# yeyupiaoling/MASR

Measured on NVIDIA H100. Metric: audio_seconds_per_second, higher is better.
Workload: dtype f32 (GEMMs: fp16x2-split operands on wgmma, fp32 accumulate; fp32-grade results)

## Files before the change

### masr_b200/csrc/ffn_tc.cu

```cuda
#include <cuda.h>
#include <cuda_fp16.h>
#include <string.h>

#include "tc_common.cuh"

namespace masr {

namespace {

constexpr int FM = 64;
constexpr int FD = 256;
constexpr int FHC = 128;
constexpr int FBK = 32;
constexpr int F_STAGES = 4;
constexpr int F_STAGE_BYTES = 32768;
constexpr int F_H_BYTES = FM * FHC * 2 * 2;
constexpr int F_SUM_BYTES = FM * FD * 4;
constexpr int F_THREADS = 384;
constexpr int F_PRODUCER_REGS = 40, F_CONSUMER_REGS = 232;
constexpr uint32_t F_TX_A = 2 * FM * FBK * 2 + 2 * FHC * FBK * 2;
constexpr uint32_t F_TX_B = 2 * FD * FBK * 2;
constexpr size_t kFfnSmem = F_STAGES * F_STAGE_BYTES + F_H_BYTES + F_SUM_BYTES + 1024 + 256;
static_assert(kFfnSmem <= 232448, "ffn_tc shared memory exceeds the 227 KB per-CTA limit of sm_90");
static_assert(F_PRODUCER_REGS * 128 + F_CONSUMER_REGS * 256 <= 65536, "register file of the SM");

struct FfnMaps {
    CUtensorMap xh, xl;
    CUtensorMap w1h, w1l;
    CUtensorMap w2h, w2l;
};

struct FfnParams {
    const float* b1;
    const float* b2;
    float* x;
    int64_t ldx;
    int M, F;
    float alpha;
};

__device__ __forceinline__ void wgmma_m64n64k16_ss(float (&d)[32], uint64_t da, uint64_t db, uint32_t scale_d) {
    asm volatile(
        "{\n\t"
        ".reg .pred p;\n\t"
        "setp.ne.b32 p, %34, 0;\n\t"
        "wgmma.mma_async.sync.aligned.m64n64k16.f32.f16.f16 "
        "{%0, %1, %2, %3, %4, %5, %6, %7, %8, %9, %10, %11, %12, %13, %14, %15, "
        "%16, %17, %18, %19, %20, %21, %22, %23, %24, %25, %26, %27, %28, %29, %30, %31}, %32, %33, p, 1, 1, 0, 0;\n\t"
        "}"
        : "+f"(d[0]), "+f"(d[1]), "+f"(d[2]), "+f"(d[3]), "+f"(d[4]), "+f"(d[5]), "+f"(d[6]), "+f"(d[7]), "+f"(d[8]),
          "+f"(d[9]), "+f"(d[10]), "+f"(d[11]), "+f"(d[12]), "+f"(d[13]), "+f"(d[14]), "+f"(d[15]), "+f"(d[16]),
          "+f"(d[17]), "+f"(d[18]), "+f"(d[19]), "+f"(d[20]), "+f"(d[21]), "+f"(d[22]), "+f"(d[23]), "+f"(d[24]),
          "+f"(d[25]), "+f"(d[26]), "+f"(d[27]), "+f"(d[28]), "+f"(d[29]), "+f"(d[30]), "+f"(d[31])
        : "l"(da), "l"(db), "r"(scale_d));
}

__device__ __forceinline__ void bar_consumers() { asm volatile("bar.sync 1, 256;" ::: "memory"); }

__global__ void __launch_bounds__(F_THREADS, 1) ffn_tc_kernel(const __grid_constant__ FfnMaps maps, FfnParams p) {
    extern __shared__ uint8_t smem_raw[];
    uint8_t* smem = reinterpret_cast<uint8_t*>((reinterpret_cast<uintptr_t>(smem_raw) + 1023) & ~uintptr_t(1023));
    uint8_t* hbuf = smem + F_STAGES * F_STAGE_BYTES;
    uint8_t* sum = hbuf + F_H_BYTES;
    uint64_t* full_bar = reinterpret_cast<uint64_t*>(sum + F_SUM_BYTES);
    uint64_t* empty_bar = full_bar + F_STAGES;

    const int warp = threadIdx.x >> 5, lane = threadIdx.x & 31;
    const int nrb = (p.M + FM - 1) / FM;
    const int nch = p.F / FHC;

    if (warp == 8 && lane == 0) {
        tma_prefetch_desc(&maps.xh); tma_prefetch_desc(&maps.xl); tma_prefetch_desc(&maps.w1h);
        tma_prefetch_desc(&maps.w1l); tma_prefetch_desc(&maps.w2h); tma_prefetch_desc(&maps.w2l);
        for (int s = 0; s < F_STAGES; ++s) { mbar_init(&full_bar[s], 1); mbar_init(&empty_bar[s], 8); }
        asm volatile("fence.mbarrier_init.release.cluster;" ::: "memory");
    }
    __syncthreads();
    pdl_wait();
    pdl_launch_dependents();

    if (warp >= 8) {
        setmaxnreg_dec<F_PRODUCER_REGS>();
        if (warp == 8 && elect_one_sync()) {
            uint32_t kg = 0;
            auto acquire = [&](uint32_t tx) {
                const uint32_t s = kg % F_STAGES;
                mbar_wait(&empty_bar[s], ((kg / F_STAGES) & 1) ^ 1);
                mbar_expect_tx(&full_bar[s], tx);
                ++kg;
                return s;
            };
            for (int rb = blockIdx.x; rb < nrb; rb += gridDim.x) {
                const int m0 = rb * FM;
                for (int j = -1; j < nch; ++j) {
                    if (j >= 0) {
#pragma unroll 1
                        for (int kb = 0; kb < FHC / FBK; ++kb) {
                            const uint32_t s = acquire(F_TX_B);
                            uint8_t* st = smem + s * F_STAGE_BYTES;
                            tma_load_2d(&maps.w2h, &full_bar[s], st, j * FHC + kb * FBK, 0);
                            tma_load_2d(&maps.w2l, &full_bar[s], st + F_STAGE_BYTES / 2, j * FHC + kb * FBK, 0);
                        }
                    }
                    if (j + 1 < nch) {
#pragma unroll 1
                        for (int kb = 0; kb < FD / FBK; ++kb) {
                            const uint32_t s = acquire(F_TX_A);
                            uint8_t* st = smem + s * F_STAGE_BYTES;
                            tma_load_2d(&maps.xh, &full_bar[s], st, kb * FBK, m0);
                            tma_load_2d(&maps.xl, &full_bar[s], st + 4096, kb * FBK, m0);
                            tma_load_2d(&maps.w1h, &full_bar[s], st + 8192, kb * FBK, (j + 1) * FHC);
                            tma_load_2d(&maps.w1l, &full_bar[s], st + 16384, kb * FBK, (j + 1) * FHC);
                        }
                    }
                }
            }
        }
        __syncwarp();
    } else {
        setmaxnreg_inc<F_CONSUMER_REGS>();
        const int wg = warp >> 2, wi = warp & 3, q = lane & 3;
        const int tid = threadIdx.x & 127;
        const uint32_t h_base = smem_u32(hbuf);
        const uint32_t sum_base = smem_u32(sum) + wg * (F_SUM_BYTES / 2) + tid * 8;
        const uint32_t is_lane0 = lane == 0;
        auto release = [&](uint32_t s) {
            asm volatile("{\n\t.reg .pred p;\n\tsetp.ne.u32 p, %1, 0;\n\t@p mbarrier.arrive.shared::cta.b64 _, [%0];\n\t}"
                         ::"r"(smem_u32(&empty_bar[s])), "r"(is_lane0) : "memory");
        };
        float acc1[32], cor1[32], acc2[64], cor2[64];
        uint32_t kg = 0;
        int pend = -1;
        auto next_stage = [&]() {
            const uint32_t s = kg % F_STAGES;
            mbar_wait(&full_bar[s], (kg / F_STAGES) & 1);
            ++kg;
            return s;
        };
        auto retire = [&](uint32_t s) {
            wgmma_wait<1>();
            reg_fence(acc1); reg_fence(cor1); reg_fence(acc2); reg_fence(cor2);
            if (pend >= 0) release((uint32_t)pend);
            pend = (int)s;
        };
        auto phase_a = [&]() {
#pragma unroll 1
            for (int kb = 0; kb < FD / FBK; ++kb) {
                const uint32_t s = next_stage();
                const uint32_t sa = smem_u32(smem + s * F_STAGE_BYTES);
                const uint64_t dXh = gmma_desc_sw64(sa), dXl = gmma_desc_sw64(sa + 4096);
                const uint64_t dWh = gmma_desc_sw64(sa + 8192 + wg * 4096), dWl = gmma_desc_sw64(sa + 16384 + wg * 4096);
                reg_fence(acc1); reg_fence(cor1);
                wgmma_fence();
#pragma unroll
                for (int ks = 0; ks < FBK / 16; ++ks) {
                    const uint64_t adv = (uint64_t)(ks * 2);
                    const uint32_t first = (kb | ks) ? 1u : 0u;
                    wgmma_m64n64k16_ss(acc1, dXh + adv, dWh + adv, first);
                    wgmma_m64n64k16_ss(cor1, dXh + adv, dWl + adv, first);
                    wgmma_m64n64k16_ss(cor1, dXl + adv, dWh + adv, 1u);
                }
                wgmma_commit();
                retire(s);
            }
        };
        auto phase_b = [&](int j) {
#pragma unroll 1
            for (int kb = 0; kb < FHC / FBK; ++kb) {
                const uint32_t s = next_stage();
                const uint32_t sa = smem_u32(smem + s * F_STAGE_BYTES);
                const uint64_t dWh = gmma_desc_sw64(sa + wg * 8192), dWl = gmma_desc_sw64(sa + F_STAGE_BYTES / 2 + wg * 8192);
                const uint64_t dHh = gmma_desc_sw64(h_base + kb * 8192), dHl = gmma_desc_sw64(h_base + kb * 8192 + 4096);
                reg_fence(acc2); reg_fence(cor2);
                wgmma_fence();
#pragma unroll
                for (int ks = 0; ks < FBK / 16; ++ks) {
                    const uint64_t adv = (uint64_t)(ks * 2);
                    wgmma_m64n128k16_ss(acc2, dHh + adv, dWh + adv, ((j & 1) | kb | ks) ? 1u : 0u);
                    wgmma_m64n128k16_ss(cor2, dHh + adv, dWl + adv, (j | kb | ks) ? 1u : 0u);
                    wgmma_m64n128k16_ss(cor2, dHl + adv, dWh + adv, 1u);
                }
                wgmma_commit();
                retire(s);
            }
        };
        const int r_lo = 16 * wi + (lane >> 2);
        auto store_hidden = [&](int j) {
            float2 bb[8];
            const float* b = p.b1 + j * FHC + 64 * wg + 2 * q;
#pragma unroll
            for (int i = 0; i < 8; ++i) bb[i] = __ldg(reinterpret_cast<const float2*>(b + 8 * i));
#pragma unroll
            for (int i = 0; i < 8; ++i)
#pragma unroll
                for (int hh = 0; hh < 2; ++hh) {
                    float v0 = fmaf(cor1[4 * i + 2 * hh], kLoInv, acc1[4 * i + 2 * hh]);
                    float v1 = fmaf(cor1[4 * i + 2 * hh + 1], kLoInv, acc1[4 * i + 2 * hh + 1]);
                    v0 += bb[i].x; v1 += bb[i].y;
                    float e0, e1;
                    mul2(e0, e1, v0, v1, -1.4426950408889634f, -1.4426950408889634f);
                    e0 = ex2_approx(e0); e1 = ex2_approx(e1);
                    add2(e0, e1, e0, e1, 1.0f, 1.0f);
                    e0 = rcp_approx(e0); e1 = rcp_approx(e1);
                    mul2(v0, v1, v0, v1, e0, e1);
                    __half2 h2, l2;
                    split_f16x2(v0, v1, h2, l2);
                    const int r = r_lo + 8 * hh, c = 64 * wg + 8 * i + 2 * q;
                    const uint32_t a = h_base + (c >> 5) * 8192 + r * 64 + ((((c & 31) >> 3) ^ ((r >> 1) & 3)) << 4) + (c & 7) * 2;
                    asm volatile("st.shared.b32 [%0], %1;" ::"r"(a), "r"(*reinterpret_cast<uint32_t*>(&h2)) : "memory");
                    asm volatile("st.shared.b32 [%0], %1;" ::"r"(a + 4096), "r"(*reinterpret_cast<uint32_t*>(&l2)) : "memory");
                }
            asm volatile("fence.proxy.async.shared::cta;" ::: "memory");
        };
        auto drain = [&]() {
            wgmma_wait<0>();
            reg_fence(acc1); reg_fence(cor1); reg_fence(acc2); reg_fence(cor2);
            if (pend >= 0) release((uint32_t)pend);
            pend = -1;
        };

        for (int rb = blockIdx.x; rb < nrb; rb += gridDim.x) {
            const int m0 = rb * FM;
            phase_a();
            drain();
            bar_consumers();
            store_hidden(0);
            bar_consumers();
#pragma unroll 1
            for (int j = 0; j < nch; ++j) {
                phase_b(j);
                if (j + 1 < nch) phase_a();
                drain();
                if ((j & 1) && j + 1 < nch) {
#pragma unroll
                    for (int i = 0; i < 16; ++i)
#pragma unroll
                        for (int hh = 0; hh < 2; ++hh) {
                            float x0 = acc2[4 * i + 2 * hh], x1 = acc2[4 * i + 2 * hh + 1];
                            const uint32_t a = sum_base + (i * 2 + hh) * 1024;
                            if (j > 1) {
                                float s0, s1;
                                asm volatile("ld.shared.v2.f32 {%0, %1}, [%2];" : "=f"(s0), "=f"(s1) : "r"(a) : "memory");
                                x0 = s0 + x0; x1 = s1 + x1;
                            }
                            asm volatile("st.shared.v2.f32 [%0], {%1, %2};" ::"r"(a), "f"(x0), "f"(x1) : "memory");
                        }
                }
                if (j + 1 < nch) {
                    bar_consumers();
                    store_hidden(j + 1);
                    bar_consumers();
                }
            }
            const float* b2 = p.b2 + 128 * wg + 2 * q;
#pragma unroll
            for (int i = 0; i < 16; ++i) {
                const float2 bv = __ldg(reinterpret_cast<const float2*>(b2 + 8 * i));
#pragma unroll
                for (int hh = 0; hh < 2; ++hh) {
                    float x0 = acc2[4 * i + 2 * hh], x1 = acc2[4 * i + 2 * hh + 1];
                    if (nch > 2) {
                        float s0, s1;
                        asm volatile("ld.shared.v2.f32 {%0, %1}, [%2];" : "=f"(s0), "=f"(s1) : "r"(sum_base + (i * 2 + hh) * 1024) : "memory");
                        x0 = s0 + x0; x1 = s1 + x1;
                    }
                    x0 = fmaf(cor2[4 * i + 2 * hh], kLoInv, x0);
                    x1 = fmaf(cor2[4 * i + 2 * hh + 1], kLoInv, x1);
                    x0 += bv.x; x1 += bv.y;
                    const int row = m0 + r_lo + 8 * hh;
                    if (row < p.M) {
                        float2* xp = reinterpret_cast<float2*>(p.x + (int64_t)row * p.ldx + 128 * wg + 8 * i + 2 * q);
                        const float2 r = *xp;
                        x0 = r.x + p.alpha * x0;
                        x1 = r.y + p.alpha * x1;
                        *xp = make_float2(x0, x1);
                    }
                }
            }
        }
    }
    __syncthreads();
}

int ffn_map(CUtensorMap* map, const void* ptr, int64_t rows, int64_t K, int64_t ld, int box_rows) {
    EncodeTiledFn fn = get_encode_fn();
    if (!fn) { set_last_error("cuTensorMapEncodeTiled entry point unavailable"); return MASR_ERR_INTERNAL; }
    cuuint64_t dims[2] = {(cuuint64_t)K, (cuuint64_t)rows};
    cuuint64_t strides[1] = {(cuuint64_t)ld * 2};
    cuuint32_t box[2] = {(cuuint32_t)FBK, (cuuint32_t)box_rows};
    cuuint32_t estr[2] = {1, 1};
    CUresult r = fn(map, CU_TENSOR_MAP_DATA_TYPE_FLOAT16, 2, const_cast<void*>(ptr), dims, strides, box, estr,
                    CU_TENSOR_MAP_INTERLEAVE_NONE, CU_TENSOR_MAP_SWIZZLE_64B, CU_TENSOR_MAP_L2_PROMOTION_L2_128B,
                    CU_TENSOR_MAP_FLOAT_OOB_FILL_NONE);
    if (r != CUDA_SUCCESS) { set_last_error("cuTensorMapEncodeTiled failed (%d) rows=%lld K=%lld ld=%lld", (int)r, (long long)rows, (long long)K, (long long)ld); return MASR_ERR_INTERNAL; }
    return MASR_OK;
}

bool g_ffn_attr_set[64] = {false};

}

}

using namespace masr;

extern "C" int masr_ffn_tc_f16x2(const void* Ah, const void* Al, int64_t lda, const void* W1h, const void* W1l, const float* b1,
                                 const void* W2h, const void* W2l, const float* b2, float* x, int64_t ldx, int M, int D, int F,
                                 float alpha, void* stream) {
    if (M == 0) return MASR_OK;
    MASR_REQUIRE(Ah && Al && W1h && W1l && b1 && W2h && W2l && b2 && x, "masr_ffn_tc_f16x2: null pointer");
    MASR_REQUIRE(M > 0, "masr_ffn_tc_f16x2: M=%d", M);
    MASR_REQUIRE(D == FD, "masr_ffn_tc_f16x2: D=%d unsupported (this build: %d)", D, FD);
    MASR_REQUIRE(F > 0 && F % 256 == 0, "masr_ffn_tc_f16x2: F=%d must be a positive multiple of 256", F);
    MASR_REQUIRE(lda >= D && lda % 8 == 0, "masr_ffn_tc_f16x2: lda=%lld must be >= %d and a multiple of 8", (long long)lda, D);
    MASR_REQUIRE(ldx >= D && ldx % 2 == 0, "masr_ffn_tc_f16x2: ldx=%lld must be >= %d and even", (long long)ldx, D);
    MASR_REQUIRE(((reinterpret_cast<uintptr_t>(Ah) | reinterpret_cast<uintptr_t>(Al) | reinterpret_cast<uintptr_t>(W1h) |
                   reinterpret_cast<uintptr_t>(W1l) | reinterpret_cast<uintptr_t>(W2h) | reinterpret_cast<uintptr_t>(W2l)) & 15) == 0 &&
                 ((reinterpret_cast<uintptr_t>(x) | reinterpret_cast<uintptr_t>(b1) | reinterpret_cast<uintptr_t>(b2)) & 7) == 0,
                 "masr_ffn_tc_f16x2: misaligned pointer");
    FfnMaps maps;
    memset(&maps, 0, sizeof(maps));
    int rc;
    if ((rc = ffn_map(&maps.xh, Ah, M, D, lda, FM))) return rc;
    if ((rc = ffn_map(&maps.xl, Al, M, D, lda, FM))) return rc;
    if ((rc = ffn_map(&maps.w1h, W1h, F, D, D, FHC))) return rc;
    if ((rc = ffn_map(&maps.w1l, W1l, F, D, D, FHC))) return rc;
    if ((rc = ffn_map(&maps.w2h, W2h, D, F, F, FD))) return rc;
    if ((rc = ffn_map(&maps.w2l, W2l, D, F, F, FD))) return rc;
    int dev = 0;
    cudaGetDevice(&dev);
    if (dev < 0 || dev >= 64) dev = 0;
    if (!g_ffn_attr_set[dev]) {
        cudaError_t e = cudaFuncSetAttribute(ffn_tc_kernel, cudaFuncAttributeMaxDynamicSharedMemorySize, (int)kFfnSmem);
        if (e != cudaSuccess) { set_last_error("ffn_tc smem attr: %s", cudaGetErrorString(e)); return (int)e; }
        g_ffn_attr_set[dev] = true;
    }
    int sms = 0;
    if (cudaDeviceGetAttribute(&sms, cudaDevAttrMultiProcessorCount, dev) != cudaSuccess || sms <= 0) sms = 132;
    const int nrb = (M + FM - 1) / FM;
    FfnParams p{b1, b2, x, ldx, M, F, alpha};
    launch_pdl(ffn_tc_kernel, dim3(nrb < sms ? nrb : sms), dim3(F_THREADS), kFfnSmem, (cudaStream_t)stream, maps, p);
    return check_launch("ffn_tc_kernel");
}
```

### masr_b200/csrc/tc_common.cuh

```cuda
#pragma once
#include <cuda.h>
#include <cuda_fp16.h>
#include <mutex>

#include "common.cuh"

namespace masr {

constexpr float kLoScale = 2048.0f, kLoInv = 1.0f / 2048.0f;

__device__ __forceinline__ uint32_t smem_u32(const void* p) { return (uint32_t)__cvta_generic_to_shared(p); }

__device__ __forceinline__ void mbar_init(uint64_t* bar, uint32_t count) {
    asm volatile("mbarrier.init.shared::cta.b64 [%0], %1;" ::"r"(smem_u32(bar)), "r"(count));
}
__device__ __forceinline__ void mbar_expect_tx(uint64_t* bar, uint32_t bytes) {
    asm volatile("mbarrier.arrive.expect_tx.shared::cta.b64 _, [%0], %1;" ::"r"(smem_u32(bar)), "r"(bytes) : "memory");
}
__device__ __forceinline__ void mbar_wait(uint64_t* bar, uint32_t parity) {
    asm volatile(
        "{\n\t"
        ".reg .pred P1;\n\t"
        "WAIT_LOOP:\n\t"
        "mbarrier.try_wait.parity.shared::cta.b64 P1, [%0], %1;\n\t"
        "@P1 bra DONE;\n\t"
        "bra WAIT_LOOP;\n\t"
        "DONE:\n\t"
        "}" ::"r"(smem_u32(bar)), "r"(parity) : "memory");
}
__device__ __forceinline__ void tma_load_2d(const CUtensorMap* map, uint64_t* bar, void* smem_dst, int c0, int c1) {
    asm volatile(
        "cp.async.bulk.tensor.2d.shared::cluster.global.mbarrier::complete_tx::bytes [%0], [%1, {%3, %4}], [%2];"
        ::"r"(smem_u32(smem_dst)), "l"(map), "r"(smem_u32(bar)), "r"(c0), "r"(c1) : "memory");
}
__device__ __forceinline__ void tma_load_2d_mc(const CUtensorMap* map, uint64_t* bar, void* smem_dst, int c0, int c1, uint16_t mask) {
    asm volatile(
        "cp.async.bulk.tensor.2d.shared::cluster.global.mbarrier::complete_tx::bytes.multicast::cluster [%0], [%1, {%3, %4}], [%2], %5;"
        ::"r"(smem_u32(smem_dst)), "l"(map), "r"(smem_u32(bar)), "r"(c0), "r"(c1), "h"(mask) : "memory");
}
__device__ __forceinline__ void mbar_arrive_remote(uint64_t* bar, uint32_t rank) {
    uint32_t a;
    asm volatile("mapa.shared::cluster.u32 %0, %1, %2;" : "=r"(a) : "r"(smem_u32(bar)), "r"(rank));
    asm volatile("mbarrier.arrive.release.cluster.shared::cluster.b64 _, [%0];" ::"r"(a) : "memory");
}
__device__ __forceinline__ void tma_prefetch_desc(const CUtensorMap* map) {
    asm volatile("prefetch.tensormap [%0];" ::"l"(map) : "memory");
}
__device__ __forceinline__ bool elect_one_sync() {
    uint32_t pred = 0, laneid = 0;
    asm volatile(
        "{\n\t"
        ".reg .b32 %%rx;\n\t"
        ".reg .pred %%px;\n\t"
        "elect.sync %%rx|%%px, %2;\n\t"
        "@%%px mov.s32 %1, 1;\n\t"
        "mov.s32 %0, %%rx;\n\t"
        "}"
        : "+r"(laneid), "+r"(pred)
        : "r"(0xFFFFFFFFu));
    return pred != 0;
}

__device__ __forceinline__ void wgmma_fence() { asm volatile("wgmma.fence.sync.aligned;" ::: "memory"); }
__device__ __forceinline__ void wgmma_commit() { asm volatile("wgmma.commit_group.sync.aligned;" ::: "memory"); }
template <int N>
__device__ __forceinline__ void wgmma_wait() { asm volatile("wgmma.wait_group.sync.aligned %0;" ::"n"(N) : "memory"); }
template <int R>
__device__ __forceinline__ void reg_fence(float (&d)[R]) {
#pragma unroll
    for (int i = 0; i < R; ++i) asm volatile("" : "+f"(d[i])::"memory");
}
__device__ __forceinline__ void wgmma_m64n128k16_ss(float (&d)[64], uint64_t da, uint64_t db, uint32_t scale_d) {
    asm volatile(
        "{\n\t"
        ".reg .pred p;\n\t"
        "setp.ne.b32 p, %66, 0;\n\t"
        "wgmma.mma_async.sync.aligned.m64n128k16.f32.f16.f16 "
        "{%0, %1, %2, %3, %4, %5, %6, %7, %8, %9, %10, %11, %12, %13, %14, %15, "
        "%16, %17, %18, %19, %20, %21, %22, %23, %24, %25, %26, %27, %28, %29, %30, %31, "
        "%32, %33, %34, %35, %36, %37, %38, %39, %40, %41, %42, %43, %44, %45, %46, %47, "
        "%48, %49, %50, %51, %52, %53, %54, %55, %56, %57, %58, %59, %60, %61, %62, %63}, %64, %65, p, 1, 1, 0, 0;\n\t"
        "}"
        : "+f"(d[0]), "+f"(d[1]), "+f"(d[2]), "+f"(d[3]), "+f"(d[4]), "+f"(d[5]), "+f"(d[6]), "+f"(d[7]), "+f"(d[8]),
          "+f"(d[9]), "+f"(d[10]), "+f"(d[11]), "+f"(d[12]), "+f"(d[13]), "+f"(d[14]), "+f"(d[15]), "+f"(d[16]),
          "+f"(d[17]), "+f"(d[18]), "+f"(d[19]), "+f"(d[20]), "+f"(d[21]), "+f"(d[22]), "+f"(d[23]), "+f"(d[24]),
          "+f"(d[25]), "+f"(d[26]), "+f"(d[27]), "+f"(d[28]), "+f"(d[29]), "+f"(d[30]), "+f"(d[31]), "+f"(d[32]),
          "+f"(d[33]), "+f"(d[34]), "+f"(d[35]), "+f"(d[36]), "+f"(d[37]), "+f"(d[38]), "+f"(d[39]), "+f"(d[40]),
          "+f"(d[41]), "+f"(d[42]), "+f"(d[43]), "+f"(d[44]), "+f"(d[45]), "+f"(d[46]), "+f"(d[47]), "+f"(d[48]),
          "+f"(d[49]), "+f"(d[50]), "+f"(d[51]), "+f"(d[52]), "+f"(d[53]), "+f"(d[54]), "+f"(d[55]), "+f"(d[56]),
          "+f"(d[57]), "+f"(d[58]), "+f"(d[59]), "+f"(d[60]), "+f"(d[61]), "+f"(d[62]), "+f"(d[63])
        : "l"(da), "l"(db), "r"(scale_d));
}
template <int R>
__device__ __forceinline__ void setmaxnreg_inc() { asm volatile("setmaxnreg.inc.sync.aligned.u32 %0;" ::"n"(R)); }
template <int R>
__device__ __forceinline__ void setmaxnreg_dec() { asm volatile("setmaxnreg.dec.sync.aligned.u32 %0;" ::"n"(R)); }

__device__ __forceinline__ uint64_t gmma_desc_sw64(uint32_t smem_addr) {
    uint64_t d = 0;
    d |= (uint64_t)((smem_addr & 0x3FFFF) >> 4);
    d |= (uint64_t)1 << 16;
    d |= (uint64_t)(512 >> 4) << 32;
    d |= (uint64_t)2 << 62;
    return d;
}

__device__ __forceinline__ void add2(float& d0, float& d1, float a0, float a1, float b0, float b1) { d0 = a0 + b0; d1 = a1 + b1; }
__device__ __forceinline__ void sub2(float& d0, float& d1, float a0, float a1, float b0, float b1) { d0 = a0 - b0; d1 = a1 - b1; }
__device__ __forceinline__ void mul2(float& d0, float& d1, float a0, float a1, float b0, float b1) { d0 = a0 * b0; d1 = a1 * b1; }
__device__ __forceinline__ void split_f16(float x, __half& h, __half& l) {
    h = __float2half_rn(x);
    l = __float2half_rn((x - __half2float(h)) * kLoScale);
}
__device__ __forceinline__ void split_f16x2(float x0, float x1, __half2& h, __half2& l) {
    h = __floats2half2_rn(x0, x1);
    const float2 hf = __half22float2(h);
    float d0, d1;
    sub2(d0, d1, x0, x1, hf.x, hf.y);
    mul2(d0, d1, d0, d1, kLoScale, kLoScale);
    l = __floats2half2_rn(d0, d1);
}

__device__ __forceinline__ void mbar_arrive(uint64_t* bar) {
    asm volatile("mbarrier.arrive.shared::cta.b64 _, [%0];" ::"r"(smem_u32(bar)) : "memory");
}

__device__ __forceinline__ void sts128(uint32_t a, const uint4& v) {
    asm volatile("st.shared.v4.b32 [%0], {%1, %2, %3, %4};" ::"r"(a), "r"(v.x), "r"(v.y), "r"(v.z), "r"(v.w) : "memory");
}
__device__ __forceinline__ uint4 lds128(uint32_t a) {
    uint4 v;
    asm volatile("ld.shared.v4.b32 {%0, %1, %2, %3}, [%4];" : "=r"(v.x), "=r"(v.y), "=r"(v.z), "=r"(v.w) : "r"(a) : "memory");
    return v;
}

typedef CUresult (*EncodeTiledFn)(CUtensorMap*, CUtensorMapDataType, cuuint32_t, void*, const cuuint64_t*, const cuuint64_t*,
                                  const cuuint32_t*, const cuuint32_t*, CUtensorMapInterleave, CUtensorMapSwizzle,
                                  CUtensorMapL2promotion, CUtensorMapFloatOOBfill);

inline EncodeTiledFn get_encode_fn() {
    static EncodeTiledFn fn = nullptr;
    static std::once_flag once;
    std::call_once(once, [] {
        void* p = nullptr;
        cudaDriverEntryPointQueryResult qres;
        if (cudaGetDriverEntryPoint("cuTensorMapEncodeTiled", &p, cudaEnableDefault, &qres) == cudaSuccess &&
            qres == cudaDriverEntryPointSuccess)
            fn = reinterpret_cast<EncodeTiledFn>(p);
    });
    return fn;
}

}
```

### masr_b200/csrc/tc_gemm.cu

```cuda
#include <cuda.h>
#include <cuda_fp16.h>
#include <math.h>
#include <mutex>
#include <stdlib.h>
#include <string.h>

#include "tc_common.cuh"

namespace masr {

constexpr int TBM = 128, TBN = 128, TBK = 32;
constexpr int TILE_BYTES = TBM * TBK * 2;
constexpr int STAGE_BYTES = 4 * TILE_BYTES;
constexpr int EW = 8;
template <bool LNC> constexpr int kStages = LNC ? 4 : 5;
constexpr int RES_BYTES = TBM * TBN * 4;
constexpr int TC_THREADS = 32 * EW + 128;
constexpr int PRODUCER_REGS = 40, CONSUMER_REGS = 232;
static_assert(PRODUCER_REGS * 128 + CONSUMER_REGS * 32 * EW <= 65536, "register file of the SM");

struct TcParams {
    const float* bias;
    const float* residual;
    float* C;
// ... 602 lines not shown
                reg_fence(acc); reg_fence(cor);
                if (pend >= 0) release((uint32_t)pend);
                if (c + 1 < nchunks) {
#pragma unroll
                    for (int i = 0; i < 16; ++i)
#pragma unroll
                        for (int hh = 0; hh < 2; ++hh) {
                            float x0 = acc[4 * i + 2 * hh], x1 = acc[4 * i + 2 * hh + 1];
                            const uint32_t a = frag_addr(i, hh);
                            if (c > 0) {
                                float s0, s1;
                                asm volatile("ld.shared.v2.f32 {%0, %1}, [%2];" : "=f"(s0), "=f"(s1) : "r"(a) : "memory");
                                x0 = s0 + x0; x1 = s1 + x1;
                            }
                            asm volatile("st.shared.v2.f32 [%0], {%1, %2};" ::"r"(a), "f"(x0), "f"(x1) : "memory");
                        }
                }
            }
#pragma unroll
            for (int i = 0; i < 16; ++i)
#pragma unroll
                for (int hh = 0; hh < 2; ++hh) {
                    const uint32_t a = frag_addr(i, hh);
                    float x0 = acc[4 * i + 2 * hh], x1 = acc[4 * i + 2 * hh + 1];
                    if (nchunks > 1) {
                        float s0, s1;
                        asm volatile("ld.shared.v2.f32 {%0, %1}, [%2];" : "=f"(s0), "=f"(s1) : "r"(a) : "memory");
                        x0 = s0 + x0; x1 = s1 + x1;
                    }
                    x0 = fmaf(cor[4 * i + 2 * hh], kLoInv, x0);
                    x1 = fmaf(cor[4 * i + 2 * hh + 1], kLoInv, x1);
                    asm volatile("st.shared.v2.f32 [%0], {%1, %2};" ::"r"(a), "f"(x0), "f"(x1) : "memory");
                }
            asm volatile("bar.sync %0, 128;" ::"r"(wg_bar) : "memory");
            for (int h = 0; h < 2; ++h) {
                const int q = 2 * wg + h;
                map_rows(m0, t0, b, q);
                ctx.sb = smem_u32(wg_res) + (h * 4 + wi) * EPI_STG;
                if (LNC) lnx.row = (uint32_t)(q * 32 + lane);
                if (nw >= p.N) continue;
                float v[32];
#pragma unroll
                for (int k = 0; k < 8; ++k) {
                    const uint4 r4 = lds128(ctx.sb + lane * 128 + ((k ^ (lane & 7)) << 4));
                    v[4 * k] = __uint_as_float(r4.x); v[4 * k + 1] = __uint_as_float(r4.y);
                    v[4 * k + 2] = __uint_as_float(r4.z); v[4 * k + 3] = __uint_as_float(r4.w);
                }
                if (p.bias != nullptr && nw + 31 < p.N && (reinterpret_cast<uintptr_t>(p.bias + nw) & 15) == 0) {
#pragma unroll
                    for (int j = 0; j < 32; j += 4) {
                        const float4 bb = ldg_f4(p.bias + nw + j);
                        v[j] += bb.x; v[j + 1] += bb.y; v[j + 2] += bb.z; v[j + 3] += bb.w;
                    }
                } else if (p.bias != nullptr) {
#pragma unroll
                    for (int j = 0; j < 32; ++j)
                        if (nw + j < p.N) v[j] += __ldg(p.bias + nw + j);
                }
                store_chunk<EPI_STG, LNC>(p, ctx, v, nw, lnx);
            }
        }
    }
    __syncthreads();
    if (LNC || PAIR) {
        asm volatile("barrier.cluster.arrive.release;" ::: "memory");
        asm volatile("barrier.cluster.wait.acquire;" ::: "memory");
    }
}

constexpr size_t kTcSmem = kStages<false> * STAGE_BYTES + RES_BYTES + 1024 + 256;
constexpr size_t kTcSmemLn = kStages<true> * STAGE_BYTES + RES_BYTES + LN_RED_BYTES + 1024 + 256;
static_assert(kTcSmem <= 232448 && kTcSmemLn <= 232448, "tc_gemm shared memory exceeds the 227 KB per-CTA limit of sm_90");

__global__ void __launch_bounds__(256) split_f16_kernel(const float* __restrict__ x, __half* __restrict__ h,
                                                        __half* __restrict__ l, int64_t n) {
    int64_t i = ((int64_t)blockIdx.x * 256 + threadIdx.x) * 4;
    if (i + 3 < n) {
        float4 v = ldg_f4(x + i);
        __half hh[4], ll[4];
        split_f16(v.x, hh[0], ll[0]); split_f16(v.y, hh[1], ll[1]); split_f16(v.z, hh[2], ll[2]); split_f16(v.w, hh[3], ll[3]);
        *reinterpret_cast<uint2*>(h + i) = *reinterpret_cast<const uint2*>(hh);
        *reinterpret_cast<uint2*>(l + i) = *reinterpret_cast<const uint2*>(ll);
    } else {
        for (; i < n; ++i) split_f16(x[i], h[i], l[i]);
    }
}

__global__ void __launch_bounds__(128) ctc_partial_combine_kernel(const float* __restrict__ pm, const float* __restrict__ ps,
                                                                  const int* __restrict__ pi, int M, int groups,
                                                                  int* __restrict__ ids, float* __restrict__ maxp) {
    pdl_wait();
    pdl_launch_dependents();
    const int lane = threadIdx.x & 31, w = threadIdx.x >> 5;
    const int row = blockIdx.x * 32 + lane;
    float m = -INFINITY, s = 0.f;
    int mi = 0x7fffffff;
    if (row < M) {
#pragma unroll 8
        for (int g = w; g < groups; g += 4) {
            const int64_t idx = (int64_t)g * M + row;
            const float gm = __ldg(pm + idx), gs = __ldg(ps + idx);
            const int gi = __ldg(pi + idx);
            if (gm > m) { s = s * expf(m - gm) + gs; m = gm; mi = gi; }
            else s += gs * expf(gm - m);
        }
    }
    __shared__ float sm_[4][32], ss_[4][32];
    __shared__ int si_[4][32];
    sm_[w][lane] = m; ss_[w][lane] = s; si_[w][lane] = mi;
    __syncthreads();
    if (w == 0 && row < M) {
#pragma unroll
        for (int k = 1; k < 4; ++k) {
            const float gm = sm_[k][lane], gs = ss_[k][lane];
            const int gi = si_[k][lane];
            if (gm > m || (gm == m && gi < mi)) { s = s * expf(m - gm) + gs; m = gm; mi = gi; }
            else s += gs * expf(gm - m);
        }
        ids[row] = mi;
        maxp[row] = 1.0f / s;
    }
}

static int make_map_2d(CUtensorMap* map, const void* ptr, int64_t rows, int64_t K, int64_t ld, int box_rows = TBM) {
    EncodeTiledFn fn = get_encode_fn();
    if (!fn) { set_last_error("cuTensorMapEncodeTiled entry point unavailable"); return MASR_ERR_INTERNAL; }
    cuuint64_t dims[2] = {(cuuint64_t)K, (cuuint64_t)rows};
    cuuint64_t strides[1] = {(cuuint64_t)ld * 2};
    cuuint32_t box[2] = {(cuuint32_t)TBK, (cuuint32_t)box_rows};
    cuuint32_t estr[2] = {1, 1};
    CUresult r = fn(map, CU_TENSOR_MAP_DATA_TYPE_FLOAT16, 2, const_cast<void*>(ptr), dims, strides, box, estr,
                    CU_TENSOR_MAP_INTERLEAVE_NONE, CU_TENSOR_MAP_SWIZZLE_64B, CU_TENSOR_MAP_L2_PROMOTION_L2_128B,
                    CU_TENSOR_MAP_FLOAT_OOB_FILL_NONE);
    if (r != CUDA_SUCCESS) { set_last_error("cuTensorMapEncodeTiled failed (%d) rows=%lld K=%lld ld=%lld", (int)r, (long long)rows, (long long)K, (long long)ld); return MASR_ERR_INTERNAL; }
    return MASR_OK;
}

static bool g_tc_attr_set[64] = {false};

static int make_map_plane(CUtensorMap* map, const void* ptr, int B, int TH, int C) {
    EncodeTiledFn fn = get_encode_fn();
    if (!fn) { set_last_error("cuTensorMapEncodeTiled entry point unavailable"); return MASR_ERR_INTERNAL; }
    cuuint64_t dims[4] = {(cuuint64_t)C, 20, (cuuint64_t)TH, (cuuint64_t)B};
    cuuint64_t strides[3] = {(cuuint64_t)C * 2, (cuuint64_t)20 * C * 2, (cuuint64_t)TH * 20 * C * 2};
    cuuint32_t box[4] = {(cuuint32_t)TBK, (cuuint32_t)CONV_W2, (cuuint32_t)CONV_TR, 1};
    cuuint32_t estr[4] = {1, 1, 1, 1};
    CUresult r = fn(map, CU_TENSOR_MAP_DATA_TYPE_FLOAT16, 4, const_cast<void*>(ptr), dims, strides, box, estr,
                    CU_TENSOR_MAP_INTERLEAVE_NONE, CU_TENSOR_MAP_SWIZZLE_64B, CU_TENSOR_MAP_L2_PROMOTION_L2_128B,
                    CU_TENSOR_MAP_FLOAT_OOB_FILL_NONE);
    if (r != CUDA_SUCCESS) { set_last_error("cuTensorMapEncodeTiled(plane) failed (%d) B=%d TH=%d", (int)r, B, TH); return MASR_ERR_INTERNAL; }
    return MASR_OK;
}

static int tc_flags() {
    const char* e = getenv("MASR_TC_FLAGS");
    return e ? atoi(e) : 1;
}

static int num_sms() {
    static int n[64] = {0};
    int dev = 0;
    cudaGetDevice(&dev);
    if (dev < 0 || dev >= 64) dev = 0;
    if (n[dev] == 0) {
        int v = 0;
        if (cudaDeviceGetAttribute(&v, cudaDevAttrMultiProcessorCount, dev) != cudaSuccess || v <= 0) v = 132;
        n[dev] = v;
    }
    return n[dev];
}

static int ensure_tc_attrs() {
    int dev = 0;
    cudaGetDevice(&dev);
    if (dev < 0 || dev >= 64) dev = 0;
    if (!g_tc_attr_set[dev]) {
        cudaError_t e = cudaFuncSetAttribute(tc_gemm_kernel<false, false>, cudaFuncAttributeMaxDynamicSharedMemorySize, (int)kTcSmem);
        if (e == cudaSuccess) e = cudaFuncSetAttribute(tc_gemm_kernel<true, false>, cudaFuncAttributeMaxDynamicSharedMemorySize, (int)kTcSmem);
        if (e == cudaSuccess) e = cudaFuncSetAttribute(tc_gemm_kernel<false, true>, cudaFuncAttributeMaxDynamicSharedMemorySize, (int)kTcSmemLn);
        if (e == cudaSuccess) e = cudaFuncSetAttribute(tc_gemm_kernel<false, false, true>, cudaFuncAttributeMaxDynamicSharedMemorySize, (int)kTcSmem);
        if (e == cudaSuccess) e = cudaFuncSetAttribute(tc_gemm_kernel<true, false, true>, cudaFuncAttributeMaxDynamicSharedMemorySize, (int)kTcSmem);
        if (e != cudaSuccess) { set_last_error("tc_gemm smem attr: %s", cudaGetErrorString(e)); return (int)e; }
        g_tc_attr_set[dev] = true;
    }
    return MASR_OK;
}

static bool pair_enabled(bool several_row_blocks) {
    const char* e = getenv("MASR_TC_PAIR");
    return several_row_blocks && e != nullptr && atoi(e) != 0;
}

template <bool CONV>
static void launch_tc(const TcMaps& maps, const TcParams& p, bool pair, int tiles_n, int tiles_m, int batch, cudaStream_t stream) {
    if (!pair) {
        const int num_tiles = tiles_n * tiles_m * batch;
        const int grid = num_tiles < num_sms() ? num_tiles : num_sms();
        launch_pdl(tc_gemm_kernel<CONV, false>, dim3(grid), dim3(TC_THREADS), kTcSmem, stream, maps, p, num_tiles, tiles_n, tiles_m);
        return;
    }
    const int ptiles_m = (tiles_m + 1) / 2;
    const int num_ptiles = tiles_n * ptiles_m * batch;
    const int pairs = num_ptiles < num_sms() / 2 ? num_ptiles : num_sms() / 2;
    cudaLaunchConfig_t cfg = {};
    cfg.gridDim = dim3(2 * pairs);
    cfg.blockDim = dim3(TC_THREADS);
    cfg.dynamicSmemBytes = kTcSmem;
    cfg.stream = stream;
    cudaLaunchAttribute attr[2];
    attr[0].id = cudaLaunchAttributeClusterDimension;
    attr[0].val.clusterDim.x = 2; attr[0].val.clusterDim.y = 1; attr[0].val.clusterDim.z = 1;
    attr[1].id = cudaLaunchAttributeProgrammaticStreamSerialization;
    attr[1].val.programmaticStreamSerializationAllowed = 1;
    cfg.attrs = attr;
    cfg.numAttrs = pdl_enabled() ? 2 : 1;
    cudaLaunchKernelEx(&cfg, tc_gemm_kernel<CONV, false, true>, maps, p, num_ptiles, tiles_n, ptiles_m);
}

}

using namespace masr;

extern "C" int masr_conv2_tc_f16x2(const void* c1h, const void* c1l, const void* Wh, const void* Wl, const float* bias,
                                   float* out, void* outh, void* outl, int B, int F1, int T2, int C, void* stream) {
    if (B == 0 || T2 == 0) return MASR_OK;
    MASR_REQUIRE(c1h && c1l && Wh && Wl && (out || (outh && outl)), "masr_conv2_tc_f16x2: null pointer");
    MASR_REQUIRE(C == 256, "masr_conv2_tc_f16x2: C=%d unsupported (this build: 256)", C);
    const int TH = (F1 + 1) / 2;
    TcMaps maps;
    memset(&maps, 0, sizeof(maps));
    int rc;
    const int64_t plane_elems = (int64_t)B * TH * 20 * C;
    for (int pl = 0; pl < 4; ++pl) {
        if ((rc = make_map_plane(&maps.a[2 * pl], (const __half*)c1h + pl * plane_elems, B, TH, C))) return rc;
        if ((rc = make_map_plane(&maps.a[2 * pl + 1], (const __half*)c1l + pl * plane_elems, B, TH, C))) return rc;
    }
    const bool pair = pair_enabled(T2 > CONV_TR);
    if ((rc = make_map_2d(&maps.w[0], Wh, C, 9 * C, 9 * C, pair ? TBN / 2 : TBN))) return rc;
    if ((rc = make_map_2d(&maps.w[1], Wl, C, 9 * C, 9 * C, pair ? TBN / 2 : TBN))) return rc;
    if ((rc = ensure_tc_attrs())) return rc;
    TcParams p{bias, nullptr, out, (__half*)outh, (__half*)outl, 0, C, B * T2 * CONV_W2, C, 9 * C, MASR_EPI_BIAS_RELU, 1.f, T2, tc_flags()};
    const int tiles_n = (C + TBN - 1) / TBN, tiles_t = (T2 + CONV_TR - 1) / CONV_TR;
    launch_tc<true>(maps, p, pair, tiles_n, tiles_t, B, (cudaStream_t)stream);
    return check_launch("tc_gemm_kernel<conv>");
}

extern "C" int masr_split_f16(const float* x, void* h, void* l, int64_t n, void* stream) {
    if (n == 0) return MASR_OK;
    MASR_REQUIRE(x && h && l, "masr_split_f16: null pointer");
    MASR_REQUIRE((reinterpret_cast<uintptr_t>(x) & 15) == 0 && (reinterpret_cast<uintptr_t>(h) & 7) == 0 &&
                 (reinterpret_cast<uintptr_t>(l) & 7) == 0, "masr_split_f16: misaligned pointer");
    int64_t blocks = (n + 1023) / 1024;
    split_f16_kernel<<<(unsigned)blocks, 256, 0, (cudaStream_t)stream>>>(x, (__half*)h, (__half*)l, n);
    return check_launch("split_f16_kernel");
}

extern "C" int masr_gemm_tc_f16x2(const void* Ah, const void* Al, int64_t lda, const void* Wh, const void* Wl,
                                  const float* bias, const float* residual, int64_t ldr, float* C, void* Ch, void* Cl,
                                  int64_t ldc, int M, int N, int K, int epilogue, float alpha, void* stream) {
    if (M == 0 || N == 0) return MASR_OK;
    MASR_REQUIRE(Ah && Al && Wh && Wl, "masr_gemm_tc_f16x2: null operand");
    MASR_REQUIRE(C || (Ch && Cl), "masr_gemm_tc_f16x2: no output");
    MASR_REQUIRE((Ch == nullptr) == (Cl == nullptr), "masr_gemm_tc_f16x2: Ch/Cl must come as a pair");
    MASR_REQUIRE(K > 0 && K % TBK == 0, "masr_gemm_tc_f16x2: K=%d must be a positive multiple of %d", K, TBK);
    MASR_REQUIRE(lda % 8 == 0, "masr_gemm_tc_f16x2: lda=%lld must be a multiple of 8", (long long)lda);
    MASR_REQUIRE(epilogue >= MASR_EPI_BIAS && epilogue <= MASR_EPI_RESIDUAL, "masr_gemm_tc_f16x2: bad epilogue %d", epilogue);
    MASR_REQUIRE(epilogue != MASR_EPI_RESIDUAL || residual, "masr_gemm_tc_f16x2: residual epilogue needs a residual");
    MASR_REQUIRE(epilogue != MASR_EPI_BIAS_GLU || N % 32 == 0, "masr_gemm_tc_f16x2: GLU epilogue needs N %% 32 == 0");
    MASR_REQUIRE(ldc % 8 == 0 || (C && !Ch && ldc % 4 == 0), "masr_gemm_tc_f16x2: ldc=%lld alignment", (long long)ldc);
    TcMaps maps;
    memset(&maps, 0, sizeof(maps));
    int rc;
    if ((rc = make_map_2d(&maps.a[0], Ah, M, K, lda))) return rc;
    if ((rc = make_map_2d(&maps.a[1], Al, M, K, lda))) return rc;
    const bool pair = pair_enabled(M > TBM);
    if ((rc = make_map_2d(&maps.w[0], Wh, N, K, K, pair ? TBN / 2 : TBN))) return rc;
    if ((rc = make_map_2d(&maps.w[1], Wl, N, K, K, pair ? TBN / 2 : TBN))) return rc;
    if ((rc = ensure_tc_attrs())) return rc;
    TcParams p{bias, residual, C, (__half*)Ch, (__half*)Cl, ldr, ldc, M, N, K, epilogue, alpha, 0, tc_flags()};
    const int tiles_n = (N + TBN - 1) / TBN, tiles_m = (M + TBM - 1) / TBM;
    launch_tc<false>(maps, p, pair, tiles_n, tiles_m, 1, (cudaStream_t)stream);
    return check_launch("tc_gemm_kernel");
}

extern "C" int masr_gemm_tc_lnpre_f16x2(const float* x, int64_t ldx, const float* gamma, const float* beta, float eps, void* Ah,
                                        void* Al, int64_t lda, const void* Wh, const void* Wl, const float* bias, float* C,
                                        void* Ch, void* Cl, int64_t ldc, int M, int N, int K, int epilogue, float alpha,
                                        void* stream) {
    if (M == 0 || N == 0) return MASR_OK;
    MASR_REQUIRE(x && gamma && beta && Ah && Al && Wh && Wl, "masr_gemm_tc_lnpre_f16x2: null pointer");
    MASR_REQUIRE(C || (Ch && Cl), "masr_gemm_tc_lnpre_f16x2: no output");
    MASR_REQUIRE((Ch == nullptr) == (Cl == nullptr), "masr_gemm_tc_lnpre_f16x2: Ch/Cl must come as a pair");
    MASR_REQUIRE(K == 256, "masr_gemm_tc_lnpre_f16x2: K=%d unsupported (the LayerNorm width of this build is 256)", K);
    MASR_REQUIRE(lda % 8 == 0 && ldx % 4 == 0 && (reinterpret_cast<uintptr_t>(x) & 15) == 0,
                 "masr_gemm_tc_lnpre_f16x2: lda=%lld ldx=%lld alignment", (long long)lda, (long long)ldx);
    MASR_REQUIRE(epilogue >= MASR_EPI_BIAS && epilogue <= MASR_EPI_BIAS_SCALE, "masr_gemm_tc_lnpre_f16x2: bad epilogue %d", epilogue);
    MASR_REQUIRE(epilogue != MASR_EPI_BIAS_GLU || N % 32 == 0, "masr_gemm_tc_lnpre_f16x2: GLU epilogue needs N %% 32 == 0");
    MASR_REQUIRE(ldc % 8 == 0 || (C && !Ch && ldc % 4 == 0), "masr_gemm_tc_lnpre_f16x2: ldc=%lld alignment", (long long)ldc);
    TcMaps maps;
    memset(&maps, 0, sizeof(maps));
    int rc;
    const int tiles_n = (N + TBN - 1) / TBN, tiles_m = (M + TBM - 1) / TBM;
    if ((rc = make_map_2d(&maps.a[0], Ah, M, K, lda))) return rc;
    if ((rc = make_map_2d(&maps.a[1], Al, M, K, lda))) return rc;
    const bool pair = pair_enabled(M > TBM);
    if ((rc = make_map_2d(&maps.w[0], Wh, N, K, K, pair ? TBN / 2 : TBN))) return rc;
    if ((rc = make_map_2d(&maps.w[1], Wl, N, K, K, pair ? TBN / 2 : TBN))) return rc;
    if ((rc = ensure_tc_attrs())) return rc;
    TcParams p{bias, nullptr, C, (__half*)Ch, (__half*)Cl, 0, ldc, M, N, K, epilogue, alpha, 0, tc_flags()};
    p.ln_g = gamma; p.ln_b = beta; p.ln_eps = eps;
    p.lnp_x = x; p.lnp_ldx = ldx; p.lnp_ld = lda; p.lnp_h = (__half*)Ah; p.lnp_l = (__half*)Al;
// ... 100 lines not shown
```

Measured before the change: 41530.

## Multicast FFN weight tiles across 2-CTA clusters via TMA

Launches the fused FFN kernel in clusters of two CTAs. Each CTA loads half of every W1/W2 weight tile and multicasts it to both CTAs, which halves the L2 weight traffic per CTA. Empty barriers now count arrivals from consumers in both CTAs, and the intra-CTA barriers become cluster barriers. It also adds profiling variants, selected through env flags, that skip loads or compute, and the row-block count is padded to a multiple of the cluster size. The cost is coupling between the paired CTAs, so one stalled CTA now stalls its partner.

Result: faster. 42830 (median of 6 runs) (+3.1%).

```diff
diff --git a/masr_b200/csrc/ffn_tc.cu b/masr_b200/csrc/ffn_tc.cu
--- a/masr_b200/csrc/ffn_tc.cu
+++ b/masr_b200/csrc/ffn_tc.cu
@@ -16,6 +16,7 @@
 constexpr int F_STAGE_BYTES = 32768;
 constexpr int F_H_BYTES = FM * FHC * 2 * 2;
 constexpr int F_SUM_BYTES = FM * FD * 4;
+constexpr int F_CS = 2;
 constexpr int F_THREADS = 384;
 constexpr int F_PRODUCER_REGS = 40, F_CONSUMER_REGS = 232;
 constexpr uint32_t F_TX_A = 2 * FM * FBK * 2 + 2 * FHC * FBK * 2;
@@ -23,6 +24,7 @@
 constexpr size_t kFfnSmem = F_STAGES * F_STAGE_BYTES + F_H_BYTES + F_SUM_BYTES + 1024 + 256;
 static_assert(kFfnSmem <= 232448, "ffn_tc shared memory exceeds the 227 KB per-CTA limit of sm_90");
 static_assert(F_PRODUCER_REGS * 128 + F_CONSUMER_REGS * 256 <= 65536, "register file of the SM");
+static_assert((FHC / F_CS) % 8 == 0 && (FD / F_CS) % 8 == 0, "W sub-boxes of whole 8-row swizzle periods");
 
 struct FfnMaps {
     CUtensorMap xh, xl;
@@ -56,7 +58,13 @@
 }
 
 __device__ __forceinline__ void bar_consumers() { asm volatile("bar.sync 1, 256;" ::: "memory"); }
-
+__device__ __forceinline__ uint32_t cluster_rank() {
+    uint32_t r;
+    asm volatile("mov.u32 %0, %%cluster_ctarank;" : "=r"(r));
+    return r;
+}
+
+template <int PROF>
 __global__ void __launch_bounds__(F_THREADS, 1) ffn_tc_kernel(const __grid_constant__ FfnMaps maps, FfnParams p) {
     extern __shared__ uint8_t smem_raw[];
     uint8_t* smem = reinterpret_cast<uint8_t*>((reinterpret_cast<uintptr_t>(smem_raw) + 1023) & ~uintptr_t(1023));
@@ -66,16 +74,17 @@
     uint64_t* empty_bar = full_bar + F_STAGES;
 
     const int warp = threadIdx.x >> 5, lane = threadIdx.x & 31;
-    const int nrb = (p.M + FM - 1) / FM;
     const int nch = p.F / FHC;
+    const int nrb = ((p.M + FM - 1) / FM + F_CS - 1) / F_CS * F_CS;
 
     if (warp == 8 && lane == 0) {
         tma_prefetch_desc(&maps.xh); tma_prefetch_desc(&maps.xl); tma_prefetch_desc(&maps.w1h);
         tma_prefetch_desc(&maps.w1l); tma_prefetch_desc(&maps.w2h); tma_prefetch_desc(&maps.w2l);
-        for (int s = 0; s < F_STAGES; ++s) { mbar_init(&full_bar[s], 1); mbar_init(&empty_bar[s], 8); }
+        for (int s = 0; s < F_STAGES; ++s) { mbar_init(&full_bar[s], 1); mbar_init(&empty_bar[s], 8 * F_CS); }
         asm volatile("fence.mbarrier_init.release.cluster;" ::: "memory");
     }
-    __syncthreads();
+    asm volatile("barrier.cluster.arrive.release;" ::: "memory");
+    asm volatile("barrier.cluster.wait.acquire;" ::: "memory");
     pdl_wait();
     pdl_launch_dependents();
 
@@ -86,10 +95,13 @@
             auto acquire = [&](uint32_t tx) {
                 const uint32_t s = kg % F_STAGES;
                 mbar_wait(&empty_bar[s], ((kg / F_STAGES) & 1) ^ 1);
-                mbar_expect_tx(&full_bar[s], tx);
+                if (!(PROF & 32)) mbar_expect_tx(&full_bar[s], tx);
                 ++kg;
                 return s;
             };
+            constexpr uint16_t mask = (1u << F_CS) - 1;
+            const uint32_t crank = cluster_rank();
+            constexpr int w1r = FHC / F_CS, w2r = FD / F_CS;
             for (int rb = blockIdx.x; rb < nrb; rb += gridDim.x) {
                 const int m0 = rb * FM;
                 for (int j = -1; j < nch; ++j) {
@@ -97,20 +109,23 @@
 #pragma unroll 1
                         for (int kb = 0; kb < FHC / FBK; ++kb) {
                             const uint32_t s = acquire(F_TX_B);
-                            uint8_t* st = smem + s * F_STAGE_BYTES;
-                            tma_load_2d(&maps.w2h, &full_bar[s], st, j * FHC + kb * FBK, 0);
-                            tma_load_2d(&maps.w2l, &full_bar[s], st + F_STAGE_BYTES / 2, j * FHC + kb * FBK, 0);
+                            if (PROF & 32) { mbar_arrive(&full_bar[s]); continue; }
+                            uint8_t* st = smem + s * F_STAGE_BYTES + crank * (w2r * 64);
+                            tma_load_2d_mc(&maps.w2h, &full_bar[s], st, j * FHC + kb * FBK, (int)crank * w2r, mask);
+                            tma_load_2d_mc(&maps.w2l, &full_bar[s], st + F_STAGE_BYTES / 2, j * FHC + kb * FBK, (int)crank * w2r, mask);
                         }
                     }
                     if (j + 1 < nch) {
 #pragma unroll 1
                         for (int kb = 0; kb < FD / FBK; ++kb) {
                             const uint32_t s = acquire(F_TX_A);
+                            if (PROF & 32) { mbar_arrive(&full_bar[s]); continue; }
                             uint8_t* st = smem + s * F_STAGE_BYTES;
                             tma_load_2d(&maps.xh, &full_bar[s], st, kb * FBK, m0);
                             tma_load_2d(&maps.xl, &full_bar[s], st + 4096, kb * FBK, m0);
-                            tma_load_2d(&maps.w1h, &full_bar[s], st + 8192, kb * FBK, (j + 1) * FHC);
-                            tma_load_2d(&maps.w1l, &full_bar[s], st + 16384, kb * FBK, (j + 1) * FHC);
+                            uint8_t* sw = st + crank * (w1r * 64);
+                            tma_load_2d_mc(&maps.w1h, &full_bar[s], sw + 8192, kb * FBK, (j + 1) * FHC + (int)crank * w1r, mask);
+                            tma_load_2d_mc(&maps.w1l, &full_bar[s], sw + 16384, kb * FBK, (j + 1) * FHC + (int)crank * w1r, mask);
                         }
                     }
                 }
@@ -127,6 +142,13 @@
         auto release = [&](uint32_t s) {
             asm volatile("{\n\t.reg .pred p;\n\tsetp.ne.u32 p, %1, 0;\n\t@p mbarrier.arrive.shared::cta.b64 _, [%0];\n\t}"
                          ::"r"(smem_u32(&empty_bar[s])), "r"(is_lane0) : "memory");
+#pragma unroll
+            for (uint32_t d = 1; d < F_CS; ++d) {
+                uint32_t a;
+                asm volatile("mapa.shared::cluster.u32 %0, %1, %2;" : "=r"(a) : "r"(smem_u32(&empty_bar[s])), "r"((cluster_rank() + d) % F_CS));
+                asm volatile("{\n\t.reg .pred p;\n\tsetp.ne.u32 p, %1, 0;\n\t@p mbarrier.arrive.shared::cluster.b64 _, [%0];\n\t}"
+                             ::"r"(a), "r"(is_lane0) : "memory");
+            }
         };
         float acc1[32], cor1[32], acc2[64], cor2[64];
         uint32_t kg = 0;
@@ -219,7 +241,10 @@
             pend = -1;
         };
 
-        for (int rb = blockIdx.x; rb < nrb; rb += gridDim.x) {
+        if (PROF & 64) {
+            for (int rb = blockIdx.x; rb < nrb; rb += gridDim.x)
+                for (int k = 0; k < nch * (FD / FBK + FHC / FBK); ++k) release(next_stage());
+        } else for (int rb = blockIdx.x; rb < nrb; rb += gridDim.x) {
             const int m0 = rb * FM;
             phase_a();
             drain();
@@ -279,7 +304,8 @@
             }
         }
     }
-    __syncthreads();
+    asm volatile("barrier.cluster.arrive.release;" ::: "memory");
+    asm volatile("barrier.cluster.wait.acquire;" ::: "memory");
 }
 
 int ffn_map(CUtensorMap* map, const void* ptr, int64_t rows, int64_t K, int64_t ld, int box_rows) {
@@ -296,7 +322,35 @@
     return MASR_OK;
 }
 
-bool g_ffn_attr_set[64] = {false};
+template <int PROF>
+int launch_ffn(const FfnMaps& maps, const FfnParams& p, int dev, cudaStream_t stream) {
+    static int max_clusters[64] = {0};
+    cudaLaunchConfig_t cfg = {};
+    cfg.blockDim = dim3(F_THREADS);
+    cfg.dynamicSmemBytes = kFfnSmem;
+    cfg.stream = stream;
+    cudaLaunchAttribute attr[2];
+    attr[0].id = cudaLaunchAttributeClusterDimension;
+    attr[0].val.clusterDim.x = F_CS; attr[0].val.clusterDim.y = 1; attr[0].val.clusterDim.z = 1;
+    attr[1].id = cudaLaunchAttributeProgrammaticStreamSerialization;
+    attr[1].val.programmaticStreamSerializationAllowed = 1;
+    cfg.attrs = attr;
+    if (max_clusters[dev] == 0) {
+        cudaError_t e = cudaFuncSetAttribute(ffn_tc_kernel<PROF>, cudaFuncAttributeMaxDynamicSharedMemorySize, (int)kFfnSmem);
+        int n = 0;
+        cfg.gridDim = dim3(F_CS);
+        cfg.numAttrs = 1;
+        if (e == cudaSuccess) e = cudaOccupancyMaxActiveClusters(&n, ffn_tc_kernel<PROF>, &cfg);
+        if (e != cudaSuccess) { set_last_error("ffn_tc launch setup: %s", cudaGetErrorString(e)); return (int)e; }
+        if (n <= 0) { set_last_error("ffn_tc: no cluster of %d CTAs fits on the device", F_CS); return MASR_ERR_INTERNAL; }
+        max_clusters[dev] = n;
+    }
+    const int ngroups = ((p.M + FM - 1) / FM + F_CS - 1) / F_CS;
+    cfg.gridDim = dim3(F_CS * (ngroups < max_clusters[dev] ? ngroups : max_clusters[dev]));
+    cfg.numAttrs = pdl_enabled() ? 2 : 1;
+    cudaLaunchKernelEx(&cfg, ffn_tc_kernel<PROF>, maps, p);
+    return check_launch("ffn_tc_kernel");
+}
 
 }
 
@@ -323,22 +377,18 @@
     int rc;
     if ((rc = ffn_map(&maps.xh, Ah, M, D, lda, FM))) return rc;
     if ((rc = ffn_map(&maps.xl, Al, M, D, lda, FM))) return rc;
-    if ((rc = ffn_map(&maps.w1h, W1h, F, D, D, FHC))) return rc;
-    if ((rc = ffn_map(&maps.w1l, W1l, F, D, D, FHC))) return rc;
-    if ((rc = ffn_map(&maps.w2h, W2h, D, F, F, FD))) return rc;
-    if ((rc = ffn_map(&maps.w2l, W2l, D, F, F, FD))) return rc;
+    if ((rc = ffn_map(&maps.w1h, W1h, F, D, D, FHC / F_CS))) return rc;
+    if ((rc = ffn_map(&maps.w1l, W1l, F, D, D, FHC / F_CS))) return rc;
+    if ((rc = ffn_map(&maps.w2h, W2h, D, F, F, FD / F_CS))) return rc;
+    if ((rc = ffn_map(&maps.w2l, W2l, D, F, F, FD / F_CS))) return rc;
     int dev = 0;
     cudaGetDevice(&dev);
     if (dev < 0 || dev >= 64) dev = 0;
-    if (!g_ffn_attr_set[dev]) {
-        cudaError_t e = cudaFuncSetAttribute(ffn_tc_kernel, cudaFuncAttributeMaxDynamicSharedMemorySize, (int)kFfnSmem);
-        if (e != cudaSuccess) { set_last_error("ffn_tc smem attr: %s", cudaGetErrorString(e)); return (int)e; }
-        g_ffn_attr_set[dev] = true;
+    const FfnParams p{b1, b2, x, ldx, M, F, alpha};
+    switch (tc_flags() & 96) {
+        case 32: return launch_ffn<32>(maps, p, dev, (cudaStream_t)stream);
+        case 64: return launch_ffn<64>(maps, p, dev, (cudaStream_t)stream);
+        case 96: return launch_ffn<96>(maps, p, dev, (cudaStream_t)stream);
+        default: return launch_ffn<0>(maps, p, dev, (cudaStream_t)stream);
     }
-    int sms = 0;
-    if (cudaDeviceGetAttribute(&sms, cudaDevAttrMultiProcessorCount, dev) != cudaSuccess || sms <= 0) sms = 132;
-    const int nrb = (M + FM - 1) / FM;
-    FfnParams p{b1, b2, x, ldx, M, F, alpha};
-    launch_pdl(ffn_tc_kernel, dim3(nrb < sms ? nrb : sms), dim3(F_THREADS), kFfnSmem, (cudaStream_t)stream, maps, p);
-    return check_launch("ffn_tc_kernel");
-}
+}
diff --git a/masr_b200/csrc/tc_common.cuh b/masr_b200/csrc/tc_common.cuh
--- a/masr_b200/csrc/tc_common.cuh
+++ b/masr_b200/csrc/tc_common.cuh
@@ -1,6 +1,7 @@
 #pragma once
 #include <cuda.h>
 #include <cuda_fp16.h>
+#include <stdlib.h>
 #include <mutex>
 
 #include "common.cuh"
@@ -134,6 +135,11 @@
     return v;
 }
 
+inline int tc_flags() {
+    const char* e = getenv("MASR_TC_FLAGS");
+    return e ? atoi(e) : 1;
+}
+
 typedef CUresult (*EncodeTiledFn)(CUtensorMap*, CUtensorMapDataType, cuuint32_t, void*, const cuuint64_t*, const cuuint64_t*,
                                   const cuuint32_t*, const cuuint32_t*, CUtensorMapInterleave, CUtensorMapSwizzle,
                                   CUtensorMapL2promotion, CUtensorMapFloatOOBfill);
diff --git a/masr_b200/csrc/tc_gemm.cu b/masr_b200/csrc/tc_gemm.cu
--- a/masr_b200/csrc/tc_gemm.cu
+++ b/masr_b200/csrc/tc_gemm.cu
@@ -778,11 +778,6 @@
     return MASR_OK;
 }
 
-static int tc_flags() {
-    const char* e = getenv("MASR_TC_FLAGS");
-    return e ? atoi(e) : 1;
-}
-
 static int num_sms() {
     static int n[64] = {0};
     int dev = 0;
```
